# Pitt-JonesLab/slam_decomposition

Hardware: AMD Instinct MI355X
Metric: Haar 2-qubit decompositions/sec (span<=3, loss<1e-8) (higher is better)
Workload: dtype f64

## Files before the change

slam_decomposition_amd/csrc/slam_device.hpp:

```cpp
#pragma once
#include <hip/hip_runtime.h>
#include <stdint.h>

#include "slam_sincos.hpp"
#include "slam_types.hpp"

namespace slamdev {

constexpr int kQuadsPerWave = 16;
constexpr int kWave = 64;
constexpr int kRow = kWave + 1;

typedef float f32x2 __attribute__((ext_vector_type(2)));
typedef float f32x4 __attribute__((ext_vector_type(4)));

template <int K, bool PSQ = false>
struct Cfg {
    static constexpr int L = K + 1;
    static constexpr int N = 6 * L;
    static constexpr int NA = (N + 3) / 4;
    static constexpr int NP = NA * 4;
    static constexpr int NBLK = NA * (NA + 1) / 2;
    static constexpr int FNEED = 20 * NA - 16;
    static constexpr int FSTRIDE = (FNEED - 4 + 31) / 32 * 32 + 4;
    static constexpr int PSP = (N + 3) / 4 * 4 + 1;
    static constexpr int TOFF = PSQ ? 6 : 0;
    static constexpr int PS0 = 12 * K + TOFF;
    static constexpr int XNEED_D = PSQ ? PS0 + 3 * PSP + N : 2 * N;
    static constexpr int XNEED_F = (kQuadsPerWave * FSTRIDE + 2 * kQuadsPerWave - 1) / (2 * kQuadsPerWave);
    static constexpr int XNEED = XNEED_D > XNEED_F ? XNEED_D : XNEED_F;
    static constexpr int XSTRIDE = PSQ ? (XNEED - 4 + 15) / 16 * 16 + 4 : (XNEED - 4 + 7) / 8 * 8 + 4;
    static constexpr int LDS_XCHG = kQuadsPerWave * XSTRIDE;
    static_assert(kQuadsPerWave * FSTRIDE * 4 <= LDS_XCHG * 8, "float overlay must fit the exchange area");
    static constexpr int LDS_FH = 2 * K * 4 * kRow * 2;
    static constexpr int LDS_DOUBLES = LDS_XCHG + LDS_FH;
    static constexpr int LDS_FH_LEAN = (K - 1) * 4 * kRow * 2;
    static constexpr int LDS_DOUBLES_LEAN = LDS_XCHG + LDS_FH_LEAN;
};

template <int K, int GC>
__host__ __device__ constexpr bool lean_layout() { return GC != 0; }
template <int K, int GC>
__host__ __device__ constexpr bool psq_layout() { return lean_layout<K, GC>() && K <= 3; }
template <int K, int GC>
__host__ __device__ constexpr int lds_work_doubles() {
    return lean_layout<K, GC>() ? Cfg<K, psq_layout<K, GC>()>::LDS_DOUBLES_LEAN : Cfg<K, false>::LDS_DOUBLES;
}
constexpr int kColdDoubles = 4;
constexpr int kSincosLdsDoubles = 2 * kSincosTableDoubles;
constexpr int kSeedRing = 8;
constexpr int kSeedRingOff = 70;
template <int K, int GC>
__host__ __device__ constexpr bool seed_ring() { return K == 1 && psq_layout<K, GC>(); }
template <int K, int GC>
__host__ __device__ constexpr int lds_doubles() { return lds_work_doubles<K, GC>() + kSincosLdsDoubles + kColdDoubles; }

__device__ const double kSinCosTable[kSincosTableDoubles] = SLAM_SINCOS_TABLE;

__device__ __forceinline__ void load_sincos_table(double2* tbl, int lane) {
    const double2 t = reinterpret_cast<const double2*>(kSinCosTable)[lane & 31];
    tbl[lane] = (lane & 32) ? make_double2(-t.x, -t.y) : t;
}

typedef const __attribute__((address_space(4))) double* gate_ptr;

__device__ __forceinline__ gate_ptr gate_matrix(const double* gates, int j) {
    unsigned long long a = (unsigned long long)(gates + 32 * j);
    asm volatile("" : "+s"(a));
    return (gate_ptr)a;
}

template <int CTRL>
__device__ __forceinline__ double dpp_f64(double v) {
    int lo = __double2loint(v), hi = __double2hiint(v);
    lo = __builtin_amdgcn_update_dpp(0, lo, CTRL, 0xF, 0xF, true);
    hi = __builtin_amdgcn_update_dpp(0, hi, CTRL, 0xF, 0xF, true);
    return __hiloint2double(hi, lo);
}
template <int CTRL>
__device__ __forceinline__ int dpp_i32(int v) {
    return __builtin_amdgcn_update_dpp(0, v, CTRL, 0xF, 0xF, true);
}
template <int CTRL>
__device__ __forceinline__ double quad_shuffle(double v) { return dpp_f64<CTRL>(v); }
__device__ __forceinline__ double quad_sum(double v) {
    v += quad_shuffle<0xB1>(v);
    v += quad_shuffle<0x4E>(v);
    return v;
}
__device__ __forceinline__ void quad_sum2(double& a, double& b) {
    const double a1 = quad_shuffle<0xB1>(a), b1 = quad_shuffle<0xB1>(b);
    a += a1; b += b1;
    const double a2 = quad_shuffle<0x4E>(a), b2 = quad_shuffle<0x4E>(b);
    a += a2; b += b2;
}
__device__ __forceinline__ double max_abs(double a, double b) {
    double m;
    asm("v_max_f64 %0, |%1|, |%2|" : "=v"(m) : "v"(a), "v"(b));
    return m;
}
__device__ __forceinline__ double quad_max(double v) {
    v = max_abs(v, quad_shuffle<0xB1>(v));
    v = max_abs(v, quad_shuffle<0x4E>(v));
    return v;
}

__device__ __forceinline__ void lds_fence() {
    __builtin_amdgcn_fence(__ATOMIC_RELEASE, "wavefront");
    __builtin_amdgcn_wave_barrier();
    __builtin_amdgcn_fence(__ATOMIC_ACQUIRE, "wavefront");
}

__device__ __forceinline__ void philox4x32_10(uint32_t c0, uint32_t c1, uint32_t c2, uint32_t c3,
                                              uint32_t k0, uint32_t k1, uint32_t (&out)[4]) {
#pragma unroll
    for (int r = 0; r < 10; ++r) {
        const uint64_t p0 = (uint64_t)0xD2511F53u * c0;
        const uint64_t p1 = (uint64_t)0xCD9E8D57u * c2;
        const uint32_t n0 = (uint32_t)(p1 >> 32) ^ c1 ^ k0;
        const uint32_t n1 = (uint32_t)p1;
        const uint32_t n2 = (uint32_t)(p0 >> 32) ^ c3 ^ k1;
        const uint32_t n3 = (uint32_t)p0;
        c0 = n0; c1 = n1; c2 = n2; c3 = n3;
        k0 += 0x9E3779B9u;
        k1 += 0xBB67AE85u;
    }
    out[0] = c0; out[1] = c1; out[2] = c2; out[3] = c3;
}

__device__ __forceinline__ double x0_from_words(uint32_t a, uint32_t b) {
    const uint64_t m = ((uint64_t)(a >> 5) << 26) + (uint64_t)(b >> 6);
    return (double)m * (1.0 / 9007199254740992.0) * 6.283185307179586476925286766559;
}
__device__ __forceinline__ double x0_philox(uint64_t seed, uint32_t target, uint32_t restart, uint32_t k,
                                            uint32_t i) {
    uint32_t w[4];
    philox4x32_10(i >> 1, restart, target, k, (uint32_t)seed, (uint32_t)(seed >> 32), w);
    return (i & 1) ? x0_from_words(w[2], w[3]) : x0_from_words(w[0], w[1]);
}

struct U3t {
    double c, s;
    double cp, sp;
    double cl, sl;
};

__device__ __forceinline__ U3t load_u3(const double* xq, int base_param) {
    const double2* t = reinterpret_cast<const double2*>(xq) + base_param;
    const double2 a = t[0], b = t[1], c = t[2];
    U3t u;
    u.c = a.x; u.s = a.y; u.cp = b.x; u.sp = b.y; u.cl = c.x; u.sl = c.y;
    return u;
}

__device__ __forceinline__ void u3_col(const U3t& t, double& f0r, double& f0i, double& f1r, double& f1i) {
    const double g1r = t.cl * f1r - t.sl * f1i;
    const double g1i = t.cl * f1i + t.sl * f1r;
    const double y0r = t.c * f0r - t.s * g1r;
    const double y0i = t.c * f0i - t.s * g1i;
    const double tr = t.s * f0r + t.c * g1r;
    const double ti = t.s * f0i + t.c * g1i;
    f0r = y0r; f0i = y0i;
    f1r = t.cp * tr - t.sp * ti;
    f1i = t.cp * ti + t.sp * tr;
}

__device__ __forceinline__ void u3_unit(const U3t& t, double f0, double f1, double& y0r, double& y0i, double& y1r, double& y1i) {
    const double g1r = t.cl * f1, g1i = t.sl * f1;
    y0r = t.c * f0 - t.s * g1r;
    y0i = -(t.s * g1i);
    const double tr = t.s * f0 + t.c * g1r;
    const double ti = t.c * g1i;
    y1r = t.cp * tr - t.sp * ti;
    y1i = t.cp * ti + t.sp * tr;
}

__device__ __forceinline__ void u3_unit_t(const U3t& t, double f0, double f1, double& y0r, double& y0i, double& y1r, double& y1i,
                                          double& tr, double& ti) {
    const double g1r = t.cl * f1, g1i = t.sl * f1;
    y0r = t.c * f0 - t.s * g1r;
    y0i = -(t.s * g1i);
    tr = t.s * f0 + t.c * g1r;
    ti = t.c * g1i;
    y1r = t.cp * tr - t.sp * ti;
    y1i = t.cp * ti + t.sp * tr;
}
__device__ __forceinline__ void l0_gate_partials(const U3t& g, double f0, double f1, double w0r, double w0i, double w1r, double w1i,
                                                 double x0r, double x0i, double x1r, double x1i, double tr, double ti, double& dth, double& dph,
                                                 double& dla) {
    const double d1r = g.cp * x0r - g.sp * x0i, d1i = g.cp * x0i + g.sp * x0r;
    dth = 0.5 * ((w1r * d1r - w1i * d1i) - (w0r * tr - w0i * ti));
    const double im1 = w1r * x1i + w1i * x1r;
    dph = -im1;
    dla = -f1 * (im1 + (w0r * x0i + w0i * x0r));
}

__device__ __forceinline__ void u3_row(const U3t& t, double& u0r, double& u0i, double& u1r, double& u1i) {
    const double g1r = t.cp * u1r - t.sp * u1i;
    const double g1i = t.cp * u1i + t.sp * u1r;
    const double n0r = t.c * u0r + t.s * g1r;
    const double n0i = t.c * u0i + t.s * g1i;
    const double tr = t.c * g1r - t.s * u0r;
    const double ti = t.c * g1i - t.s * u0i;
    u0r = n0r; u0i = n0i;
    u1r = t.cl * tr - t.sl * ti;
    u1i = t.cl * ti + t.sl * tr;
}

__device__ __forceinline__ void u3_row_t(const U3t& t, double& u0r, double& u0i, double& u1r, double& u1i, double& tr,
                                         double& ti) {
    const double g1r = t.cp * u1r - t.sp * u1i;
    const double g1i = t.cp * u1i + t.sp * u1r;
    const double n0r = t.c * u0r + t.s * g1r;
    const double n0i = t.c * u0i + t.s * g1i;
    tr = t.c * g1r - t.s * u0r;
    ti = t.c * g1i - t.s * u0i;
    u0r = n0r; u0i = n0i;
    u1r = t.cl * tr - t.sl * ti;
    u1i = t.cl * ti + t.sl * tr;
}
__device__ __forceinline__ void dtheta_dlam_last(const U3t& g, double n0r, double n0i, double tr, double ti, double f0r, double f0i,
                                                 double f1r, double f1i, double& dth, double& dlam) {
    const double gr = g.cl * f1r - g.sl * f1i, gi = g.cl * f1i + g.sl * f1r;
    dth = 0.5 * ((tr * f0r - ti * f0i) - (n0r * gr - n0i * gi));
    dlam = -(tr * gi + ti * gr);
}

__device__ __forceinline__ void dtheta_dlam_last_real(const U3t& g, double n0r, double n0i, double tr, double ti, double f0, double f1,
                                                      double& dth, double& dlam) {
    const double gr = g.cl * f1, gi = g.sl * f1;
    dth = 0.5 * (tr * f0 - (n0r * gr - n0i * gi));
    dlam = -(tr * gi + ti * gr);
}

__device__ __forceinline__ void u3_row_dtheta_first(const U3t& t, double& u0r, double& u0i, double& u1r, double& u1i, double h0r,
                                                    double h0i, double h1r, double h1i, double& dth2) {
    const double g1r = t.cp * u1r - t.sp * u1i;
    const double g1i = t.cp * u1i + t.sp * u1r;
    const double pr = u0r * h1r - u0i * h1i, pi = u0r * h1i + u0i * h1r;
    dth2 += (g1r * h0r - g1i * h0i) - (t.cp * pr + t.sp * pi);
    const double n0r = t.c * u0r + t.s * g1r;
    const double n0i = t.c * u0i + t.s * g1i;
    const double tr = t.c * g1r - t.s * u0r;
    const double ti = t.c * g1i - t.s * u0i;
    u0r = n0r; u0i = n0i;
    u1r = t.cl * tr - t.sl * ti;
    u1i = t.cl * ti + t.sl * tr;
}

__device__ __forceinline__ double dtheta_pair(const U3t& t, double ut0r, double ut0i, double ut1r, double ut1i,
                                              double f0r, double f0i, double f1r, double f1i) {
    const double ar = ut1r * f0r - ut1i * f0i, ai = ut1r * f0i + ut1i * f0r;
    const double br = ut0r * f1r - ut0i * f1i, bi = ut0r * f1i + ut0i * f1r;
    return 0.5 * ((t.cl * ar + t.sl * ai) - (t.cl * br - t.sl * bi));
}

__device__ __forceinline__ double im_mul(double ar, double ai, double br, double bi) { return ar * bi + ai * br; }

__device__ __forceinline__ double fast_rcp(double x) {
    double r = __builtin_amdgcn_rcp(x);
    r = fma(fma(-x, r, 1.0), r, r);
    r = fma(fma(-x, r, 1.0), r, r);
    return r;
}
__device__ __forceinline__ double fast_rsqrt(double x) {
    double y = __builtin_amdgcn_rsq(x);
    y = fma(0.5 * y, fma(-x * y, y, 1.0), y);
    y = fma(0.5 * y, fma(-x * y, y, 1.0), y);
    return y;
}

__device__ __forceinline__ void u3_arrived(const U3t& a, const U3t& b) {
    asm volatile("" ::"v"(a.c), "v"(a.s), "v"(a.cp), "v"(a.sp), "v"(a.cl), "v"(a.sl), "v"(b.c), "v"(b.s), "v"(b.cp), "v"(b.sp),
                 "v"(b.cl), "v"(b.sl));
}
__device__ __forceinline__ void vec_arrived(const double (&r)[4], const double (&i)[4]) {
    asm volatile("" ::"v"(r[0]), "v"(r[1]), "v"(r[2]), "v"(r[3]), "v"(i[0]), "v"(i[1]), "v"(i[2]), "v"(i[3]));
}

__device__ __attribute__((noinline)) void sincos_slow(double x, double* s, double* c) { sincos(x, s, c); }

__device__ __forceinline__ void sincos_any(double x, const double2* tbl, double& s, double& c) {
    if (__builtin_expect(fabs(x) < kSincosTblLimit, 1)) {
        sincos_tbl(x, tbl, s, c);
    } else {
        sincos_slow(x, &s, &c);
    }
}

enum : int { GC_DENSE = 0, GC_XGEN = 1, GC_XRI = 2, GC_CX = 3, GC_XRI1 = 4 };

#define SLAM_GRE(r, s) G[((r) * 4 + (s)) * 2]
#define SLAM_GIM(r, s) G[((r) * 4 + (s)) * 2 + 1]

template <int R0, int R1>
__device__ __forceinline__ void block_col_gen(gate_ptr G, double (&Fr)[4], double (&Fi)[4]) {
    const double ar = Fr[R0], ai = Fi[R0], br = Fr[R1], bi = Fi[R1];
    Fr[R0] = fma(SLAM_GRE(R0, R0), ar, fma(-SLAM_GIM(R0, R0), ai, fma(SLAM_GRE(R0, R1), br, -SLAM_GIM(R0, R1) * bi)));
    Fi[R0] = fma(SLAM_GRE(R0, R0), ai, fma(SLAM_GIM(R0, R0), ar, fma(SLAM_GRE(R0, R1), bi, SLAM_GIM(R0, R1) * br)));
    Fr[R1] = fma(SLAM_GRE(R1, R0), ar, fma(-SLAM_GIM(R1, R0), ai, fma(SLAM_GRE(R1, R1), br, -SLAM_GIM(R1, R1) * bi)));
    Fi[R1] = fma(SLAM_GRE(R1, R0), ai, fma(SLAM_GIM(R1, R0), ar, fma(SLAM_GRE(R1, R1), bi, SLAM_GIM(R1, R1) * br)));
}
template <int R0, int R1>
__device__ __forceinline__ void block_row_gen(gate_ptr G, double (&Ur)[4], double (&Ui)[4]) {
    const double ar = Ur[R0], ai = Ui[R0], br = Ur[R1], bi = Ui[R1];
    Ur[R0] = fma(ar, SLAM_GRE(R0, R0), fma(-ai, SLAM_GIM(R0, R0), fma(br, SLAM_GRE(R1, R0), -bi * SLAM_GIM(R1, R0))));
    Ui[R0] = fma(ar, SLAM_GIM(R0, R0), fma(ai, SLAM_GRE(R0, R0), fma(br, SLAM_GIM(R1, R0), bi * SLAM_GRE(R1, R0))));
    Ur[R1] = fma(ar, SLAM_GRE(R0, R1), fma(-ai, SLAM_GIM(R0, R1), fma(br, SLAM_GRE(R1, R1), -bi * SLAM_GIM(R1, R1))));
    Ui[R1] = fma(ar, SLAM_GIM(R0, R1), fma(ai, SLAM_GRE(R0, R1), fma(br, SLAM_GIM(R1, R1), bi * SLAM_GRE(R1, R1))));
}
template <int R0, int R1>
__device__ __forceinline__ void block_col_ri(gate_ptr G, double (&Fr)[4], double (&Fi)[4]) {
    const double d0 = SLAM_GRE(R0, R0), o01 = SLAM_GIM(R0, R1), o10 = SLAM_GIM(R1, R0), d1 = SLAM_GRE(R1, R1);
    const double ar = Fr[R0], ai = Fi[R0], br = Fr[R1], bi = Fi[R1];
    Fr[R0] = fma(d0, ar, -o01 * bi);
    Fi[R0] = fma(d0, ai, o01 * br);
    Fr[R1] = fma(d1, br, -o10 * ai);
    Fi[R1] = fma(d1, bi, o10 * ar);
}
template <int R0, int R1>
__device__ __forceinline__ void block_row_ri(gate_ptr G, double (&Ur)[4], double (&Ui)[4]) {
    const double d0 = SLAM_GRE(R0, R0), o01 = SLAM_GIM(R0, R1), o10 = SLAM_GIM(R1, R0), d1 = SLAM_GRE(R1, R1);
    const double ar = Ur[R0], ai = Ui[R0], br = Ur[R1], bi = Ui[R1];
    Ur[R0] = fma(d0, ar, -o10 * bi);
    Ui[R0] = fma(d0, ai, o10 * br);
    Ur[R1] = fma(d1, br, -o01 * ai);
    Ui[R1] = fma(d1, bi, o01 * ar);
}

template <int GC>
__device__ __forceinline__ void gate_col(gate_ptr G, double (&Fr)[4], double (&Fi)[4]) {
    if constexpr (GC == GC_CX) {
        const double tr = Fr[1], ti = Fi[1];
        Fr[1] = Fr[3]; Fi[1] = Fi[3];
        Fr[3] = tr; Fi[3] = ti;
    } else if constexpr (GC == GC_XRI1) {
        block_col_ri<1, 2>(G, Fr, Fi);
    } else if constexpr (GC == GC_XRI) {
        block_col_ri<0, 3>(G, Fr, Fi);
        block_col_ri<1, 2>(G, Fr, Fi);
    } else if constexpr (GC == GC_XGEN) {
        block_col_gen<0, 3>(G, Fr, Fi);
        block_col_gen<1, 2>(G, Fr, Fi);
    } else {
        double nr[4], ni[4];
#pragma unroll
        for (int r = 0; r < 4; ++r) {
            double ar = 0.0, ai = 0.0;
#pragma unroll
            for (int s = 0; s < 4; ++s) {
                const double gx = SLAM_GRE(r, s), gy = SLAM_GIM(r, s);
                ar = fma(gx, Fr[s], fma(-gy, Fi[s], ar));
                ai = fma(gx, Fi[s], fma(gy, Fr[s], ai));
            }
            nr[r] = ar; ni[r] = ai;
        }
// ... 776 lines not shown
```

slam_decomposition_amd/csrc/slam_kernels.hpp:

```cpp
#pragma once
#include "slam_device.hpp"

namespace slamdev {

constexpr double kArmijoC1 = 1e-4;
constexpr int kMaxBacktrack = 20;
constexpr double kStepMax = 2.0;
constexpr double kCurvEps = 1e-10;
constexpr double kStallDf = 1e-15;
constexpr double kStallGnorm = 1e-5;
constexpr double kWolfeC2 = 0.7;
constexpr double kGrowFactor = 8.0;
constexpr double kGrowMax = 1048576.0;
constexpr int kRestartPeriod = 128;
static_assert((kRestartPeriod & (kRestartPeriod - 1)) == 0, "the periodic restart tests iters & (period - 1)");

__device__ __forceinline__ unsigned long long pack2(int lo, int hi) { return (unsigned long long)(unsigned)lo | ((unsigned long long)(unsigned)hi << 32); }
__device__ __forceinline__ void item_rec_store(ItemRec* r, double loss, int iters, int status, int evals, int acc) {
    r->loss = loss;
    asm volatile("" ::: "memory");
    r->iters = iters;
    asm volatile("" ::: "memory");
    r->status = status;
    asm volatile("" ::: "memory");
    r->evals = evals;
    asm volatile("" ::: "memory");
    r->acc = acc;
    asm volatile("" ::: "memory");
    *reinterpret_cast<int2*>(&r->pad[0]) = make_int2(0, 0);
}
__device__ __forceinline__ void item_rec_store_dropped(ItemRec* r, int status) { item_rec_store(r, (double)INFINITY, 0, status, 0, 0); }

enum : int { ST_CONVERGED = 0, ST_MAXITER = 1, ST_LINESEARCH = 2, ST_NONFINITE = 3, ST_STALLED = 4, ST_PREEMPTED = 5 };


constexpr uint32_t kFlagTrace = 0x100u;
constexpr uint32_t kFlagNoExterior = 0x200u;

template <int K>
struct MinimizeArgs {
    const double* targets;
    const int32_t* orig;
    int32_t first_target;
    const double* x0;
    StageCtl* ctl;
    int32_t restarts;
    int32_t maxiter;
    double gtol;
    double stop_loss;
    double gtol_far;
    double far_loss;
    double exit_loss;
    uint64_t seed;
    int64_t target_base;
    uint32_t flags;
    uint32_t items_per_quad;
    int32_t cost_kind;
    int32_t* solved;
    ItemRec* item_rec;
    double* item_x;
    const double* gates;
    double* trace_loss;
    double* trace_x;
    int32_t trace_cap;
};

template <int K>
struct EvalArgs {
    const double* targets;
    const double* x;
    const int32_t* target_of;
    int64_t n_items;
    double* loss;
    double* grad;
    double* unitary;
    int32_t cost_kind;
    const double* gates;
};

template <int K, int GC, bool MK>
__device__ __forceinline__ void eval_body(const EvalArgs<K>& args) {
    using C = Cfg<K, psq_layout<K, GC>()>;
    extern __shared__ __attribute__((aligned(16))) double lds[];
    double* xchg = lds;
    double2* fhbase = reinterpret_cast<double2*>(lds + C::LDS_XCHG);
    const int lane = threadIdx.x;
    const int q = lane & 3;
    const int quad = lane >> 2;
    double2* tbl = reinterpret_cast<double2*>(lds + lds_work_doubles<K, GC>());
    load_sincos_table(tbl, lane);
    lds_fence();
    const int64_t item = (int64_t)blockIdx.x * kQuadsPerWave + quad;
    const bool live = item < args.n_items;
    const int64_t it = live ? item : 0;
    const int64_t tgt = args.target_of[it];
    const double* tcol = args.targets + tgt * 32 + q * 2;
    double xd[C::NA], gd[C::NA];
#pragma unroll
    for (int a = 0; a < C::NA; ++a) {
        const int i = 4 * a + q;
        xd[a] = (i < C::N) ? args.x[it * C::N + i] : 0.0;
    }
    double f, Wr[4], Wi[4];
    if constexpr (MK) {
        double gT[3];
        mk_target_g(tcol, q, gT);
        eval_quad<K, true, GC, true>(xd, tcol, args.gates, xchg + quad * C::XSTRIDE, fhbase + lane, tbl, q, theta_slot_bits<K>(q), args.cost_kind, f, gd,
                                     Wr, Wi, gT);
    } else {
        eval_quad<K, true, GC>(xd, tcol, args.gates, xchg + quad * C::XSTRIDE, fhbase + lane, tbl, q, theta_slot_bits<K>(q), args.cost_kind, f, gd, Wr, Wi);
    }
    if (live) {
        if (q == 0) args.loss[item] = f;
        if (args.unitary) {
#pragma unroll
            for (int r = 0; r < 4; ++r) {
                args.unitary[item * 32 + (r * 4 + q) * 2] = Wr[r];
                args.unitary[item * 32 + (r * 4 + q) * 2 + 1] = Wi[r];
            }
        }
        if (args.grad) {
#pragma unroll
            for (int a = 0; a < C::NA; ++a) {
                const int i = 4 * a + q;
                if (i < C::N) args.grad[item * C::N + i] = gd[a];
            }
        }
    }
}
template <int K, int GC>
__global__ void __launch_bounds__(kWave) eval_kernel(EvalArgs<K> args) {
    eval_body<K, GC, false>(args);
}
template <int K>
__global__ void __launch_bounds__(kWave) eval_mk_kernel(EvalArgs<K> args) {
    eval_body<K, GC_DENSE, true>(args);
}

template <int K>
__device__ __forceinline__ const __attribute__((address_space(4))) MinimizeArgs<K>* cold_args() {
    unsigned long long a = (unsigned long long)__builtin_amdgcn_kernarg_segment_ptr();
    asm volatile("" : "+s"(a));
    return (const __attribute__((address_space(4))) MinimizeArgs<K>*)a;
}
template <int K, bool MQ>
__device__ __forceinline__ const __attribute__((address_space(4))) MinimizeArgs<K>* cold_args(unsigned long long cur) {
    if constexpr (MQ) {
        unsigned lo = (unsigned)__builtin_amdgcn_readfirstlane((int)(unsigned)cur), hi = (unsigned)__builtin_amdgcn_readfirstlane((int)(unsigned)(cur >> 32));
        unsigned long long u = ((unsigned long long)hi << 32) | lo;
        asm volatile("" : "+s"(u));
        return (const __attribute__((address_space(4))) MinimizeArgs<K>*)u;
    } else {
        return cold_args<K>();
    }
}

struct WlStage {
    int t;
    int* flag;
    double* win_x;
    double win_loss;
    int win_r;
    bool hit;
    unsigned ev_all, ev_acc, ev_pre;
    unsigned rounds;
    unsigned round_cap;
};
__device__ __forceinline__ double readlane_f64(double v, int l) {
    const int lo = __builtin_amdgcn_readlane(__double2loint(v), l), hi = __builtin_amdgcn_readlane(__double2hiint(v), l);
    return __hiloint2double(hi, lo);
}

template <int K, int GC, bool MQ, bool WL, bool MK = false>
__device__ __forceinline__ void minimize_body(const MinimizeArgs<K>& args, const MinimizeArgs<K>* subs, int n_sub, WlStage& wl) {
    static_assert(!WL || MQ, "the wave-local stage reads its argument block from device memory");
    static_assert(!MK || (!MQ && GC == GC_DENSE), "MakhlinFunctionalCost: per-span launches of the dense gate class only");
    using C = Cfg<K, psq_layout<K, GC>()>;
    constexpr int NA = C::NA;
    extern __shared__ __attribute__((aligned(16))) double lds[];
    double* xchg = lds;
    double2* fhbase = reinterpret_cast<double2*>(lds + C::LDS_XCHG);
    const int lane = threadIdx.x;
    int q = lane & 3;
    const int quad = lane >> 2;
    const int theta_bits = theta_slot_bits<K>(q);
    double* xq = xchg + quad * C::XSTRIDE;
    float* xq32 = reinterpret_cast<float*>(xchg) + quad * C::FSTRIDE;
    double2* fh = fhbase + lane;
    double2* tbl = reinterpret_cast<double2*>(lds + lds_work_doubles<K, GC>());
    load_sincos_table(tbl, lane);
    double2* cold = tbl + kSincosLdsDoubles / 2;
    if (lane == 0) {
        cold[0] = make_double2(args.gtol, args.stop_loss);
        cold[1] = make_double2(args.gtol_far, args.far_loss);
    }
    lds_fence();
    constexpr bool kRing = seed_ring<K, GC>();
    if constexpr (kRing) static_assert(kSeedRingOff + C::N <= C::XSTRIDE && kSeedRingOff >= C::XNEED && (kSeedRingOff & 1) == 0, "the ring slots sit in the spare part of a quad's exchange area");
    double* const ring = xchg + 8 * C::XSTRIDE + kSeedRingOff;
    unsigned ring_base = 0, ring_end = 0;
    unsigned sub_idx = MQ ? (unsigned)blockIdx.x % (unsigned)n_sub : 0u;
    unsigned long long cur = MQ ? (unsigned long long)(subs + sub_idx) : 0ull;
    int sub_tries = 0;
    unsigned n_act = WL ? 1u : (unsigned)(MQ ? cold_args<K, MQ>(cur)->ctl->n_active : args.ctl->n_active);
    unsigned n_items = n_act * (unsigned)args.restarts;
    unsigned n_waves = (n_items + kQuadsPerWave - 1) / kQuadsPerWave;
    if constexpr (WL) {
        n_waves = 1;
    } else if constexpr (!MQ) {
        if (args.items_per_quad > 1) {
            n_waves = (n_items + kQuadsPerWave * args.items_per_quad - 1) / (kQuadsPerWave * args.items_per_quad);
            if (n_waves < 1 && n_items) n_waves = 1;
        }
        if (n_waves > gridDim.x) n_waves = gridDim.x;
        if (blockIdx.x >= n_waves) return;
    } else {
        n_waves = gridDim.x / (unsigned)n_sub + 1u;
    }
    unsigned kChunkV;
    {
        const unsigned per_wave = n_items / n_waves;
        kChunkV = per_wave >= 256u ? 64u : (per_wave >= 64u ? 32u : 16u);
    }

    bool live = false, fresh = false, scaled = false;
    unsigned item = 0;
    int slot = 0, tgt = 0;
    int nev = 0, iters = 0, nback = 0, nstall = 0, status = ST_MAXITER;
    double f = 0.0, alpha = 0.0, gp = 0.0, gnorm = 0.0, grow = 1.0;
    double pp = 0.0, hs1 = 0.0;
    const double* tcol = cold_args<K, MQ>(cur)->targets + q * 2;
    double x[NA], g[NA], p[NA];
#pragma unroll
    for (int a = 0; a < NA; ++a) { x[a] = 0.0; g[a] = 0.0; p[a] = 0.0; }
    HMat<NA> H;
    h_set_identity_where<NA>(H, q, true);
    double mkt[3] = {0.0, 0.0, 0.0};
    bool exhausted = false;
    const unsigned kChunk = kChunkV;
    unsigned cur_next = 0, cur_end = WL ? n_items : 0u;
    unsigned pre_base = 0;
    unsigned rounds = 0;
    if constexpr (!WL) {
        if (lane == 0) pre_base = atomicAdd(&cold_args<K, MQ>(cur)->ctl->work_counter, kChunk);
    }

    while (true) {
        if constexpr (MQ && !WL) {
            if (exhausted && !__any(live)) {
                if (lane == 0 && rounds) atomicAdd(&cold_args<K, MQ>(cur)->ctl->rounds, (unsigned long long)rounds);
                rounds = 0;
                if (++sub_tries >= n_sub) break;
                sub_idx = (sub_idx + 1u == (unsigned)n_sub) ? 0u : sub_idx + 1u;
                cur = (unsigned long long)(subs + sub_idx);
                n_act = (unsigned)cold_args<K, MQ>(cur)->ctl->n_active;
                n_items = n_act * (unsigned)args.restarts;
                exhausted = false;
                cur_next = 0;
                cur_end = 0;
                ring_base = 0;
                ring_end = 0;
                if (lane == 0) pre_base = atomicAdd(&cold_args<K, MQ>(cur)->ctl->work_counter, kChunk);
            }
        }
        if constexpr (K == 2) {
            asm volatile("" : "+v"(q));
            __builtin_assume((unsigned)q < 4u);
        }
        bool taken = false;
        {
#ifndef SLAM_REFILL_BATCH_K1
#define SLAM_REFILL_BATCH_K1 2
#endif
#ifndef SLAM_REFILL_BATCH_K2
#define SLAM_REFILL_BATCH_K2 1
#endif
            constexpr int kRefillBatch = (K == 1) ? SLAM_REFILL_BATCH_K1 : (K == 2 ? SLAM_REFILL_BATCH_K2 : 1);
            const int n_idle = __popcll(__ballot(!live && q == 0));
            const bool go = n_idle >= kRefillBatch || n_idle == __popcll(__ballot(q == 0));
            while (go && !exhausted && __any(!live)) {
                if constexpr (WL) {
                    if (cur_next >= cur_end) { exhausted = true; break; }
                } else if (cur_next >= cur_end) {
                    const unsigned b = (unsigned)__builtin_amdgcn_readfirstlane((int)pre_base);
                    cur_next = b;
                    cur_end = (b + kChunk < n_items) ? b + kChunk : n_items;
                    if (b >= n_items) { exhausted = true; break; }
                    if constexpr (MQ) sub_tries = 0;
                    if (lane == 0) pre_base = atomicAdd(&cold_args<K, MQ>(cur)->ctl->work_counter, kChunk);
                }
                bool use_ring = false;
                if constexpr (kRing) {
                    use_ring = cold_args<K, MQ>(cur)->x0 == nullptr;
                    if (use_ring && cur_next >= ring_end) {
                        constexpr int kPairs = C::N / 2;
                        ring_base = cur_next;
                        ring_end = (cur_next + (unsigned)kSeedRing < cur_end) ? cur_next + (unsigned)kSeedRing : cur_end;
                        const int gr_ = lane / kPairs, gm = lane - gr_ * kPairs;
                        if ((unsigned)gr_ < ring_end - ring_base) {
                            const unsigned gp = ring_base + (unsigned)gr_;
                            const unsigned grs = gp / n_act, gsl = gp - grs * n_act;
                            int gt_;
                            if constexpr (WL) gt_ = wl.t;
                            else gt_ = cold_args<K, MQ>(cur)->orig ? cold_args<K, MQ>(cur)->orig[gsl] : cold_args<K, MQ>(cur)->first_target + (int)gsl;
                            const uint64_t gseed = cold_args<K, MQ>(cur)->seed;
                            uint32_t w[4];
                            philox4x32_10((uint32_t)gm, grs, (uint32_t)(gt_ + (int)cold_args<K, MQ>(cur)->target_base), (uint32_t)K, (uint32_t)gseed,
                                          (uint32_t)(gseed >> 32), w);
                            *reinterpret_cast<double2*>(ring + gr_ * C::XSTRIDE + 2 * gm) = make_double2(x0_from_words(w[0], w[1]), x0_from_words(w[2], w[3]));
                        }
                        lds_fence();
                    }
                }
                unsigned wlen = (cur_end - cur_next < (unsigned)kWave) ? cur_end - cur_next : (unsigned)kWave;
                if (kRing && use_ring && ring_end - cur_next < wlen) wlen = ring_end - cur_next;
                const bool valid = (unsigned)lane < wlen;
                const unsigned pos = cur_next + (unsigned)lane;
                const unsigned prs = pos / n_act;
                const unsigned psl = pos - prs * n_act;
                bool skipv = false;
                if ((args.flags & 1u) && valid) {
                    int fl;
                    if constexpr (WL) fl = *reinterpret_cast<volatile int*>(wl.flag);
                    else fl = __hip_atomic_load(&(MQ ? cold_args<K, MQ>(cur)->solved : args.solved)[psl], __ATOMIC_RELAXED, __HIP_MEMORY_SCOPE_AGENT);
                    const int mine = args.restarts - (int)prs;
                    skipv = (args.flags & 2u) ? (fl > mine) : (fl != 0);
                }
                const unsigned long long lt = (1ull << lane) - 1ull;
                const unsigned long long avail = __ballot(valid && !skipv);
                const unsigned long long idle = __ballot(!live && q == 0);
                const int n_av = __popcll(avail), n_idle_now = __popcll(idle);
                const int n_take = n_av < n_idle_now ? n_av : n_idle_now;
                const int myrank = __popcll(avail & lt);
                const bool handed = valid && !skipv && myrank < n_take;
                const unsigned long long handed_mask = __ballot(handed);
                const unsigned consumed = (n_take == n_av) ? wlen : (unsigned)(64 - __builtin_clzll(handed_mask));
                if constexpr (!WL) {
                    if (valid && skipv && (unsigned)lane < consumed) {
                        const unsigned o = psl * (unsigned)args.restarts + prs;
                        item_rec_store_dropped(cold_args<K, MQ>(cur)->item_rec + o, ST_PREEMPTED);
                    }
                }
                int* wp = reinterpret_cast<int*>(xchg);
                if (handed) {
                    wp[myrank] = (int)psl;
                    wp[16 + myrank] = (int)prs;
                    if constexpr (kRing) wp[32 + myrank] = (int)(pos - ring_base);
                }
                lds_fence();
                const int qrank = __popcll(idle & ((1ull << (lane & ~3)) - 1ull));
                const bool get = !live && qrank < n_take;
                const unsigned sl = get ? (unsigned)wp[qrank] : 0u;
                const unsigned rs = get ? (unsigned)wp[16 + qrank] : 0u;
                const int rslot = (kRing && get) ? wp[32 + qrank] : 0;
                lds_fence();
                cur_next += consumed;
                {
                    constexpr bool kSharedSeeds = psq_layout<K, GC>();
                    const bool shared = kSharedSeeds && cold_args<K, MQ>(cur)->x0 == nullptr;
                    if (get) {
                        const unsigned oidx = sl * (unsigned)args.restarts + rs;
                        item = oidx;
                        slot = (int)sl;
                        const unsigned restart = rs;
                        if constexpr (WL) {
                            tgt = wl.t;
                            tcol = cold_args<K, MQ>(cur)->targets + (int64_t)wl.t * 32 + q * 2;
                        } else {
                            tgt = cold_args<K, MQ>(cur)->orig ? cold_args<K, MQ>(cur)->orig[sl] : cold_args<K, MQ>(cur)->first_target + (int)sl;
                            tcol = cold_args<K, MQ>(cur)->targets + (int64_t)sl * 32 + q * 2;
                        }
                        if (!shared) {
#pragma unroll
                            for (int a = 0; a < NA; ++a) {
                                const int i = 4 * a + q;
                                double xv = 0.0;
                                if (i < C::N) {
                                    if constexpr (kSharedSeeds)
                                        xv = cold_args<K, MQ>(cur)->x0[(int64_t)oidx * C::N + i];
                                    else
                                        xv = cold_args<K, MQ>(cur)->x0 ? cold_args<K, MQ>(cur)->x0[(int64_t)oidx * C::N + i]
                                                     : x0_philox(cold_args<K, MQ>(cur)->seed, (uint32_t)(tgt + (int)cold_args<K, MQ>(cur)->target_base), restart, (uint32_t)K, (uint32_t)i);
                                }
                                x[a] = xv;
                            }
                        }
#pragma unroll
                        for (int a = 0; a < NA; ++a) {
                            p[a] = 0.0;
                            g[a] = 0.0;
                        }
                        alpha = 0.0; gp = 0.0; f = 0.0; grow = 1.0; pp = 0.0; hs1 = 0.0;
                        nev = 0; iters = 0; nback = 0; nstall = 0; status = ST_MAXITER;
                        scaled = false; fresh = true; live = true; taken = true;
                        h_set_identity<NA>(H, q);
                    }
                    if constexpr (kRing) {
                        if (shared && get) {
#pragma unroll
                            for (int a = 0; a < NA; ++a) x[a] = (4 * a + q < C::N) ? ring[rslot * C::XSTRIDE + 4 * a + q] : 0.0;
                        }
                    } else if constexpr (kSharedSeeds) {
                        if (shared) {
                            constexpr int kPairs = C::N / 2;
                            static_assert(5 * C::N <= C::XSTRIDE && 4 * C::N * 8 >= 64 * 4, "staging area [4N, 5N) inside the quad's exchange area and clear of wp");
                            if (get && q == 0) {
                                wp[32 + qrank] = tgt + (int)cold_args<K, MQ>(cur)->target_base;
                                wp[48 + qrank] = quad;
                            }
                            lds_fence();
                            const uint64_t seed = cold_args<K, MQ>(cur)->seed;
                            const int jobs = n_take * kPairs;
                            for (int j0 = 0; j0 < jobs; j0 += kWave) {
                                const int jb = j0 + lane;
                                if (jb < jobs) {
                                    const int r = jb / kPairs, m = jb - r * kPairs;
                                    uint32_t w[4];
                                    philox4x32_10((uint32_t)m, (uint32_t)wp[16 + r], (uint32_t)wp[32 + r], (uint32_t)K, (uint32_t)seed,
                                                  (uint32_t)(seed >> 32), w);
                                    *reinterpret_cast<double2*>(xchg + wp[48 + r] * C::XSTRIDE + 4 * C::N + 2 * m) =
                                        make_double2(x0_from_words(w[0], w[1]), x0_from_words(w[2], w[3]));
                                }
                            }
                            lds_fence();
                            if (get) {
#pragma unroll
                                for (int a = 0; a < NA; ++a) x[a] = (4 * a + q < C::N) ? xq[4 * C::N + 4 * a + q] : 0.0;
                            }
                            lds_fence();
                        }
                    }
                    if ((args.flags & kFlagNoExterior) && get) {
#pragma unroll
                        for (int a = 0; a < NA; ++a) {
                            const int i = 4 * a + q;
                            x[a] = (i < 6 || i >= 6 * K) ? 0.0 : x[a];
                        }
                    }
                }
            }
            if constexpr (MK) {
                if (__any(taken)) {
                    double g3[3];
                    mk_target_g(tcol, q, g3);
#pragma unroll
                    for (int i = 0; i < 3; ++i) mkt[i] = taken ? g3[i] : mkt[i];
                }
            }
        }
        if (!__any(live)) {
            if constexpr (MQ && !WL) continue;
            else break;
        }
        if constexpr (WL) {
            if (rounds >= wl.round_cap) break;
        }
        ++rounds;

        int sflag = 0;
        if (args.flags & 1u) {
            if constexpr (WL) sflag = *reinterpret_cast<volatile int*>(wl.flag);
            else sflag = __hip_atomic_load(&(MQ ? cold_args<K, MQ>(cur)->solved : args.solved)[slot], __ATOMIC_RELAXED, __HIP_MEMORY_SCOPE_AGENT);
        }

        double gt[NA];
        double ft, Wr[4], Wi[4];
        {
            double xt[NA];
#pragma unroll
            for (int a = 0; a < NA; ++a) xt[a] = fma(alpha, p[a], x[a]);
            if constexpr (MK) {
                eval_quad<K, false, GC, true>(xt, tcol, args.gates, xq, fh, tbl, q, theta_bits, 0, ft, gt, Wr, Wi, mkt);
            } else {
                eval_quad<K, false, GC>(xt, tcol, MQ ? cold_args<K, MQ>(cur)->gates : args.gates, xq, fh, tbl, q, theta_bits,
                                        WL ? __builtin_amdgcn_readfirstlane(args.cost_kind) : args.cost_kind, ft, gt, Wr, Wi);
            }
        }
        const bool active = live;
        const bool finite = isfinite(ft);
#pragma unroll
        for (int a = 0; a < NA; ++a) gt[a] = finite ? gt[a] : 0.0;
        if (args.flags & kFlagNoExterior) {
#pragma unroll
            for (int a = 0; a < NA; ++a) {
                const int i = 4 * a + q;
                gt[a] = (i < 6 || i >= 6 * K) ? 0.0 : gt[a];
            }
        }
        const bool armijo = finite && (ft <= f + kArmijoC1 * alpha * gp);
        const bool acc = active && (fresh ? finite : armijo);
        const bool step = acc && !fresh;
        nev += active ? (acc ? 0x100001 : 1) : 0;

        const double am = step ? alpha : 0.0;
        double qv[NA];
        __builtin_amdgcn_sched_barrier(0);
        h_matvec<NA>(H, gt, xq32, q, qv);
        __builtin_amdgcn_sched_barrier(0);
        double pgt = 0.0, yy = 0.0;
#pragma unroll
        for (int a = 0; a < NA; ++a) {
            const double ya = gt[a] - g[a];
            pgt = fma(p[a], gt[a], pgt);
            yy = fma(ya, ya, yy);
        }
        quad_sum2(pgt, yy);
        const double sg = am * pgt;
        const double sy = am * (pgt - gp);
        const double ss = (am * am) * pp;
        const bool too_short = sy < (1.0 - kWolfeC2) * alpha * (-gp);
        const bool curv = step && !too_short && sy > 0.0 && (sy * sy > (kCurvEps * kCurvEps) * (ss * yy));
        const bool first = curv && !scaled;
        scaled = scaled || curv;
        const double fac = first ? (sy * fast_rcp(yy)) : 1.0;
        hs1 = first ? fac - 1.0 : hs1;
        double yu = 0.0;
#pragma unroll
        for (int a = 0; a < NA; ++a) {
            qv[a] = fma(hs1, gt[a], qv[a]);
            const double ua = fma(fac, p[a], qv[a]);
            yu = fma(gt[a] - g[a], ua, yu);
        }
        yu = quad_sum(yu);
        const double rho = curv ? fast_rcp(sy) : 0.0;
        const double cf = rho * (1.0 + rho * yu);
        double wg = 0.0;
        {
            float s32[NA], w32[NA], v32[NA];
#pragma unroll
            for (int a = 0; a < NA; ++a) {
                const double sa = am * p[a];
                const double ua = fma(fac, p[a], qv[a]);
                const double wa = cf * sa - rho * ua;
                const double va = -rho * ua;
                s32[a] = (float)sa;
                w32[a] = (float)wa;
                v32[a] = (float)va;
                wg = fma(wa, gt[a], wg);
            }
            __builtin_amdgcn_sched_barrier(0);
            h_update<NA>(H, s32, w32, v32, xq32, q);
            __builtin_amdgcn_sched_barrier(0);
        }
        wg = quad_sum(wg);
        const double2 th0 = cold[0], th1 = cold[1];
        __builtin_amdgcn_sched_barrier(0);

#pragma unroll
        for (int a = 0; a < NA; ++a) x[a] += am * p[a];
        bool done = false;
        if (acc) {
            nstall = (step && (f - ft) <= kStallDf) ? nstall + 1 : 0;
            f = ft;
            if (step) ++iters;
            nback = 0;
            grow = (step && too_short) ? fmin(grow * kGrowFactor, kGrowMax) : 1.0;
#pragma unroll
            for (int a = 0; a < NA; ++a) {
                const double sa = am * p[a];
                const double ua = fma(fac, p[a], qv[a]);
                const double va = -rho * ua;
                g[a] = gt[a];
                p[a] = -(qv[a] + sa * wg + va * sg);
            }
            if (args.flags & kFlagTrace) {
                const auto* ca = cold_args<K, MQ>(cur);
                const int t_cap = ca->trace_cap;
                double* const t_loss = ca->trace_loss;
                double* const t_x = ca->trace_x;
                if (step && iters <= t_cap) {
                const int64_t row = (int64_t)item * t_cap + (iters - 1);
                if (q == 0) t_loss[row] = f;
#pragma unroll
                for (int a = 0; a < NA; ++a) {
                    const int i = 4 * a + q;
                    if (i < C::N) t_x[row * C::N + i] = x[a];
                }
                }
            }
        } else if (active) {
            if (fresh) {
                f = ft;
                status = ST_NONFINITE;
                done = true;
            } else {
                const double denom = 2.0 * (ft - f - gp * alpha);
                const double anew = (finite && denom > 0.0 && isfinite(denom)) ? (-gp * alpha * alpha * fast_rcp(denom)) : 0.5 * alpha;
                alpha = fmin(fmax(anew, 0.1 * alpha), 0.5 * alpha);
                grow = 1.0;
                ++nback;
            }
        }
        {
            double m = max_abs(g[0], g[NA > 1 ? 1 : 0]);
#pragma unroll
            for (int a = 2; a < NA; ++a) m = max_abs(m, g[a]);
            gnorm = quad_max(m);
        }
        gp = qdot<NA>(g, p);
        pp = qdot<NA>(p, p);
        if (acc) {
            alpha = (pp > 1e-300) ? fmin(grow, kStepMax * fast_rsqrt(pp)) : grow;
            if (f < th0.y || gnorm < th0.x || (gnorm < th1.x && f > th1.y)) {
                status = ST_CONVERGED; done = true;
            } else if (nstall >= 2) { status = ST_STALLED; done = true; }
            else if (iters >= args.maxiter) { status = ST_MAXITER; done = true; }
        } else if (active && !fresh) {
            if (nback > kMaxBacktrack) { status = (gnorm < kStallGnorm) ? ST_STALLED : ST_LINESEARCH; done = true; }
        }
        fresh = false;
        const bool periodic = step && !done && ((iters & (kRestartPeriod - 1)) == 0);
        const bool reset = active && !done && (!(gp < 0.0) || periodic);
        if (__any(reset)) {
            h_set_identity_where<NA>(H, q, reset);
            hs1 = reset ? 0.0 : hs1;
            scaled = periodic ? false : scaled;
#pragma unroll
            for (int a = 0; a < NA; ++a) p[a] = reset ? -g[a] : p[a];
            const double gg2 = qdot<NA>(g, g);
            gp = reset ? -gg2 : gp;
            pp = reset ? gg2 : pp;
            alpha = periodic ? ((gg2 > 1e-300) ? fmin(grow, kStepMax * fast_rsqrt(gg2)) : grow) : alpha;
        }
        if (args.flags & 1u) {
            asm volatile("" : "+v"(sflag));
            const int mine = args.restarts - (int)(item - (unsigned)slot * (unsigned)args.restarts);
            const bool beaten = (args.flags & 2u) ? (sflag > mine) : (sflag != 0);
            if (active && !done && beaten) { status = ST_PREEMPTED; done = true; }
            if (active && done && status != ST_PREEMPTED && f < args.exit_loss && q == 0) {
                if constexpr (WL) __hip_atomic_fetch_max(wl.flag, mine, __ATOMIC_RELAXED, __HIP_MEMORY_SCOPE_WORKGROUP);
                else __hip_atomic_fetch_max(&(MQ ? cold_args<K, MQ>(cur)->solved : args.solved)[slot], mine, __ATOMIC_RELAXED, __HIP_MEMORY_SCOPE_AGENT);
            }
        }
        if constexpr (WL) {
            const bool fin = active && done;
            if (fin && q == 0) {
                const unsigned e = (unsigned)(nev & 0xFFFFF);
                wl.ev_all += e;
                if (status == ST_PREEMPTED) wl.ev_pre += e;
                else wl.ev_acc += (unsigned)nev >> 20;
            }
            unsigned long long m = __ballot(fin && q == 0 && status != ST_PREEMPTED);
            while (m) {
                const int l = __builtin_ctzll(m);
                m &= m - 1ull;
                const double lf = readlane_f64(f, l);
                const int lr = __builtin_amdgcn_readlane((int)item, l);
                const bool below = lf < args.exit_loss;
                const bool take = wl.hit ? (below && lr < wl.win_r) : (below || lf < wl.win_loss || (lf == wl.win_loss && lr < wl.win_r));
                if (take) {
                    wl.win_loss = lf;
                    wl.win_r = lr;
                    wl.hit = wl.hit || below;
                    if ((lane >> 2) == (l >> 2)) {
#pragma unroll
                        for (int a = 0; a < NA; ++a)
                            if (4 * a + q < C::N) wl.win_x[4 * a + q] = x[a];
                    }
                }
            }
            if (fin) {
                live = false;
                alpha = 0.0;
            }
        } else if (active && done) {
            if (q == 0) item_rec_store(cold_args<K, MQ>(cur)->item_rec + item, f, iters, status, nev & 0xFFFFF, (int)((unsigned)nev >> 20));
#pragma unroll
            for (int a = 0; a < NA; ++a) {
                const int i = 4 * a + q;
                if (i < C::N) cold_args<K, MQ>(cur)->item_x[(int64_t)item * C::N + i] = x[a];
            }
            live = false;
            alpha = 0.0;
        }
    }
    if constexpr (WL) {
        wl.rounds = rounds;
        lds_fence();
    } else if constexpr (!MQ) {
        if (lane == 0 && rounds) atomicAdd(&cold_args<K>()->ctl->rounds, (unsigned long long)rounds);
    }
}

template <int K, int GC, bool MQ = false>
__global__ void __launch_bounds__(kWave, (K <= 2 ? 2 : 1)) minimize_kernel(MinimizeArgs<K> args, const MinimizeArgs<K>* subs, int n_sub) {
    WlStage none{};
    minimize_body<K, GC, MQ, false>(args, subs, n_sub, none);
}
template <int K>
__global__ void __launch_bounds__(kWave, (K <= 2 ? 2 : 1)) minimize_mk_kernel(MinimizeArgs<K> args) {
    WlStage none{};
    minimize_body<K, GC_DENSE, false, false, true>(args, nullptr, 0, none);
}

struct WaveLoopArgs {
    const MinimizeArgs<1>* stage_args;
    StageCtl* ctl;
    int32_t k_min, k_max;
    int32_t first, count;
    double threshold;
    double* best_loss;
    double* best_x;
    int32_t* best_cycles;
// ... 481 lines not shown
```

Before: 4.673 million.

## Park pre-generated Philox seeds in registers for K=2 shared-seed refills

Result: no change. 4.709 million (median of 6 runs) (+0.8%).

```diff
diff --git a/slam_decomposition_amd/csrc/slam_device.hpp b/slam_decomposition_amd/csrc/slam_device.hpp
--- a/slam_decomposition_amd/csrc/slam_device.hpp
+++ b/slam_decomposition_amd/csrc/slam_device.hpp
@@ -52,6 +52,8 @@
 constexpr int kSeedRingOff = 70;
 template <int K, int GC>
 __host__ __device__ constexpr bool seed_ring() { return K == 1 && psq_layout<K, GC>(); }
+template <int K, int GC>
+__host__ __device__ constexpr bool seed_park() { return K == 2 && psq_layout<K, GC>(); }
 template <int K, int GC>
 __host__ __device__ constexpr int lds_doubles() { return lds_work_doubles<K, GC>() + kSincosLdsDoubles + kColdDoubles; }
 
diff --git a/slam_decomposition_amd/csrc/slam_kernels.hpp b/slam_decomposition_amd/csrc/slam_kernels.hpp
--- a/slam_decomposition_amd/csrc/slam_kernels.hpp
+++ b/slam_decomposition_amd/csrc/slam_kernels.hpp
@@ -199,6 +199,11 @@
     if constexpr (kRing) static_assert(kSeedRingOff + C::N <= C::XSTRIDE && kSeedRingOff >= C::XNEED && (kSeedRingOff & 1) == 0, "the ring slots sit in the spare part of a quad's exchange area");
     double* const ring = xchg + 8 * C::XSTRIDE + kSeedRingOff;
     unsigned ring_base = 0, ring_end = 0;
+    constexpr bool kPark = seed_park<K, GC>();
+    constexpr int kParkPairs = C::N / 2, kParkPos = kWave / kParkPairs;
+    static_assert(!kPark || !kRing, "one way of keeping start points per span");
+    double2 park = make_double2(0.0, 0.0);
+    unsigned park_pos = ~0u;
     unsigned sub_idx = MQ ? (unsigned)blockIdx.x % (unsigned)n_sub : 0u;
     unsigned long long cur = MQ ? (unsigned long long)(subs + sub_idx) : 0ull;
     int sub_tries = 0;
@@ -260,6 +265,7 @@
                 cur_end = 0;
                 ring_base = 0;
                 ring_end = 0;
+                park_pos = ~0u;
                 if (lane == 0) pre_base = atomicAdd(&cold_args<K, MQ>(cur)->ctl->work_counter, kChunk);
             }
         }
@@ -330,7 +336,12 @@
                 const unsigned long long avail = __ballot(valid && !skipv);
                 const unsigned long long idle = __ballot(!live && q == 0);
                 const int n_av = __popcll(avail), n_idle_now = __popcll(idle);
-                const int n_take = n_av < n_idle_now ? n_av : n_idle_now;
+                int n_take = n_av < n_idle_now ? n_av : n_idle_now;
+                bool use_park = false;
+                if constexpr (kPark) {
+                    use_park = cold_args<K, MQ>(cur)->x0 == nullptr;
+                    if (use_park && n_take > kParkPos) n_take = kParkPos;
+                }
                 const int myrank = __popcll(avail & lt);
                 const bool handed = valid && !skipv && myrank < n_take;
                 const unsigned long long handed_mask = __ballot(handed);
@@ -342,17 +353,55 @@
                     }
                 }
                 int* wp = reinterpret_cast<int*>(xchg);
-                if (handed) {
+                const int qrank = __popcll(idle & ((1ull << (lane & ~3)) - 1ull));
+                const bool get = !live && qrank < n_take;
+                const int pgrp = lane / kParkPairs, pm = lane - pgrp * kParkPairs;
+                unsigned prel = park_pos - cur_next;
+                bool pdeal = false;
+                bool gen = false;
+                if constexpr (kPark) {
+                    if (use_park) {
+                        pdeal = park_pos != ~0u && prel < (unsigned)kWave && ((handed_mask >> prel) & 1ull);
+                        gen = __popcll(__ballot(pdeal && pm == 0)) != n_take;
+                    }
+                }
+                if (gen ? (valid && !skipv && myrank < kParkPos) : handed) {
                     wp[myrank] = (int)psl;
                     wp[16 + myrank] = (int)prs;
                     if constexpr (kRing) wp[32 + myrank] = (int)(pos - ring_base);
+                    if constexpr (kPark) wp[32 + myrank] = (int)pos;
+                }
+                if constexpr (kPark) {
+                    if (get && q == 0) wp[48 + qrank] = quad;
                 }
                 lds_fence();
-                const int qrank = __popcll(idle & ((1ull << (lane & ~3)) - 1ull));
-                const bool get = !live && qrank < n_take;
                 const unsigned sl = get ? (unsigned)wp[qrank] : 0u;
                 const unsigned rs = get ? (unsigned)wp[16 + qrank] : 0u;
                 const int rslot = (kRing && get) ? wp[32 + qrank] : 0;
+                if constexpr (kPark) {
+                    static_assert(!kPark || (5 * C::N <= C::XSTRIDE && 4 * C::N * 8 >= 64 * 4), "staging area [4N, 5N) inside the quad's exchange area and clear of wp");
+                    if (gen) {
+                        const int n_gen = n_av < kParkPos ? n_av : kParkPos;
+                        const bool gv = pgrp < n_gen;
+                        const unsigned gsl = gv ? (unsigned)wp[pgrp] : 0u;
+                        const unsigned grs = gv ? (unsigned)wp[16 + pgrp] : 0u;
+                        park_pos = gv ? (unsigned)wp[32 + pgrp] : ~0u;
+                        int gt_;
+                        if constexpr (WL) gt_ = wl.t;
+                        else gt_ = cold_args<K, MQ>(cur)->orig ? cold_args<K, MQ>(cur)->orig[gsl] : cold_args<K, MQ>(cur)->first_target + (int)gsl;
+                        const uint64_t gseed = cold_args<K, MQ>(cur)->seed;
+                        uint32_t w[4];
+                        philox4x32_10((uint32_t)pm, grs, (uint32_t)(gt_ + (int)cold_args<K, MQ>(cur)->target_base), (uint32_t)K, (uint32_t)gseed,
+                                      (uint32_t)(gseed >> 32), w);
+                        park = make_double2(x0_from_words(w[0], w[1]), x0_from_words(w[2], w[3]));
+                        prel = park_pos - cur_next;
+                        pdeal = gv && prel < (unsigned)kWave && ((handed_mask >> prel) & 1ull);
+                    }
+                    if (pdeal) {
+                        const int tq = wp[48 + __popcll(avail & ((1ull << prel) - 1ull))];
+                        *reinterpret_cast<double2*>(xchg + tq * C::XSTRIDE + 4 * C::N + 2 * pm) = park;
+                    }
+                }
                 lds_fence();
                 cur_next += consumed;
                 {
@@ -399,6 +448,14 @@
                         if (shared && get) {
 #pragma unroll
                             for (int a = 0; a < NA; ++a) x[a] = (4 * a + q < C::N) ? ring[rslot * C::XSTRIDE + 4 * a + q] : 0.0;
+                        }
+                    } else if constexpr (kPark) {
+                        if (shared) {
+                            if (get) {
+#pragma unroll
+                                for (int a = 0; a < NA; ++a) x[a] = (4 * a + q < C::N) ? xq[4 * C::N + 4 * a + q] : 0.0;
+                            }
+                            lds_fence();
                         }
                     } else if constexpr (kSharedSeeds) {
                         if (shared) {
```
